# SonSang/dmesh2_renderer

Measured on AMD Instinct MI355X. Metric: Mpixels/s fwd+bwd @1080p/1M tris, higher is better.
Workload: dtype f32

## Files before the change

### dmesh2_renderer_amd/csrc/dm2_binning.hip

```cpp
#include <hip/hip_runtime.h>

#include <cstdlib>
#include <cstring>
#include <rocprim/rocprim.hpp>

#include "dm2_device_math.h"
#include "dm2_pairs.h"
#include "dm2_stage.h"
#include "dm2_state.h"

namespace dm2 {

__global__ void __launch_bounds__(256) k_zero_words(uint32_t* __restrict__ p, int64_t n) {
    const int64_t i = (int64_t)blockIdx.x * blockDim.x + threadIdx.x;
    if (i < n) p[i] = 0u;
}
static void launch_zero_words(void* p, int64_t n, hipStream_t st) {
    if (n > 0) hipLaunchKernelGGL(k_zero_words, dim3((unsigned)((n + 255) / 256)), dim3(256), 0, st, (uint32_t*)p, n);
}

struct TilePlace { uint32_t base; int leader; uint32_t offset; };
__device__ __forceinline__ bool wave_tiles_shared(uint32_t t, bool act) {
    const unsigned long long all = __ballot(act);
    if (all == 0) return false;
    const int l0 = __ffsll((long long)all) - 1;
    const unsigned long long m0 = __ballot(act && t == (uint32_t)__builtin_amdgcn_readlane((int)t, l0));
    return __popcll(m0) * 8 > __popcll(all);
}
template <bool RANK, int STRIDE>
__device__ __forceinline__ TilePlace wave_count_tiles_issue(uint32_t* cnt, uint32_t t, bool act, bool grouped) {
    const int lane = (int)__builtin_amdgcn_mbcnt_hi(~0u, __builtin_amdgcn_mbcnt_lo(~0u, 0u));
    TilePlace p; p.base = 0u; p.leader = lane; p.offset = 0u;
    const unsigned long long all = __ballot(act);
    if (all == 0) return p;
    if (!grouped) {
        if (act) { if (RANK) p.base = atomicAdd(cnt + (int64_t)STRIDE * t, 1u); else atomicAdd(cnt + (int64_t)STRIDE * t, 1u); }
        return p;
    }
    unsigned long long todo = all, mine = 0;
    while (todo) {
        const int l = __ffsll((long long)todo) - 1;
        const uint32_t tl = (uint32_t)__builtin_amdgcn_readlane((int)t, l);
        const unsigned long long m = __ballot(act && t == tl);
        if (act && t == tl) mine = m;
        todo &= ~m;
    }
    p.leader = act ? __ffsll((long long)mine) - 1 : lane;
    if (act && lane == p.leader) {
        if (RANK) p.base = atomicAdd(cnt + (int64_t)STRIDE * t, (uint32_t)__popcll(mine));
        else atomicAdd(cnt + (int64_t)STRIDE * t, (uint32_t)__popcll(mine));
    }
    p.offset = (uint32_t)__popcll(mine & ((1ull << lane) - 1ull));
    return p;
}
__device__ __forceinline__ uint32_t wave_count_tiles_finish(const TilePlace& p) {
    return (uint32_t)__shfl((int)p.base, p.leader) + p.offset;
}
template <bool RANK, int STRIDE>
__device__ __forceinline__ uint32_t wave_count_tiles(uint32_t* cnt, uint32_t t, bool act) {
    const TilePlace p = wave_count_tiles_issue<RANK, STRIDE>(cnt, t, act, wave_tiles_shared(t, act));
    return RANK ? wave_count_tiles_finish(p) : 0u;
}

enum { PRE_LAYERS = 0,
       PRE_FUSED = 1 };
__host__ __device__ constexpr int pre_items(int) { return 1; }

__device__ __forceinline__ void store_records(const FaceRec& r, bool has, unsigned long long tmask, int64_t idx, uint4* __restrict__ recs, uint4* sw) {
    const uint4* src = reinterpret_cast<const uint4*>(&r);
    const int lane = (int)(threadIdx.x & 63);
    uint4* dst = recs + (idx - lane) * FACE_REC_U4;
#pragma unroll
    for (int half = 0; half < 2; half++) {
        if (has) {
#pragma unroll
            for (int k = 0; k < 8; k++) sw[lane * 8 + (k ^ (lane & 7))] = src[half * 8 + k];
        }
        __builtin_amdgcn_fence(__ATOMIC_SEQ_CST, "wavefront");
#pragma unroll
        for (int j = 0; j < 8; j++) {
            const int rr = j * 8 + (lane >> 3), c = lane & 7;
            if ((tmask >> rr) & 1ull) dst[(int64_t)rr * FACE_REC_U4 + half * 8 + c] = sw[rr * 8 + (c ^ (rr & 7))];
        }
        __builtin_amdgcn_fence(__ATOMIC_SEQ_CST, "wavefront");
    }
}

#ifndef DM2_PRE_WAVES
#define DM2_PRE_WAVES 1
#endif
template <int MODE>
__global__ void __launch_bounds__(256, DM2_PRE_WAVES)
k_preprocess(int B, int P, int F, uint32_t gx, uint32_t gy, uint32_t block_stride, const int32_t* __restrict__ patch_min,
             const int32_t* __restrict__ faces, const float* __restrict__ verts_ndc,
             const float* __restrict__ verts_image, FaceState fs, dm2_render_desc d) {
    constexpr bool PACK = MODE == PRE_FUSED;
    constexpr int DM2_PRE_ITEMS = pre_items(MODE);
    const int64_t BF = (int64_t)B * F;
    int64_t idx_[DM2_PRE_ITEMS]; int vid_[DM2_PRE_ITEMS][3]; float2 img_[DM2_PRE_ITEMS][3];
#pragma unroll
    for (int it = 0; it < DM2_PRE_ITEMS; it++) {
        const uint32_t chunk = (uint32_t)(((uint64_t)blockIdx.x * block_stride) % gridDim.x);
        idx_[it] = ((int64_t)chunk * DM2_PRE_ITEMS + it) * 256 + threadIdx.x;
        const int64_t ic = idx_[it] < BF ? idx_[it] : BF - 1;
        const int f = (int)(ic % F);
        vid_[it][0] = faces[3 * f]; vid_[it][1] = faces[3 * f + 1]; vid_[it][2] = faces[3 * f + 2];
    }
#pragma unroll
    for (int it = 0; it < DM2_PRE_ITEMS; it++) {
        const int64_t ic = idx_[it] < BF ? idx_[it] : BF - 1;
        const float* img = verts_image + (ic / F) * P * 2;
#pragma unroll
        for (int k = 0; k < 3; k++) img_[it][k] = *reinterpret_cast<const float2*>(img + 2 * vid_[it][k]);
    }
#pragma unroll
    for (int it = 0; it < DM2_PRE_ITEMS; it++) {
    const bool valid = idx_[it] < BF;
    if (!__ballot(valid)) break;
    const int64_t idx = valid ? idx_[it] : BF - 1;
    const int b = (int)(idx / F), f = (int)(idx % F);
    const uint32_t pmx = patch_min ? (uint32_t)patch_min[2 * b] : 0u, pmy = patch_min ? (uint32_t)patch_min[2 * b + 1] : 0u;
    const int v0 = vid_[it][0], v1 = vid_[it][1], v2 = vid_[it][2];
    const float* ndc = verts_ndc + (int64_t)b * P * 3;
    const float2 i0 = img_[it][0], i1 = img_[it][1], i2 = img_[it][2];

    uint32_t touched = 0, lo = 0, hi = 0;
    float d01 = 0.f, dmin = 0.f, dmax = 0.f;
    {
        uint32_t x0, y0, x1, y1;
        patch_rect_from_tri(pmx, pmy, i0.x, i0.y, i1.x, i1.y, i2.x, i2.y, gx, gy, x0, y0, x1, y1);
        touched = valid ? (y1 - y0) * (x1 - x0) : 0u;
        if (touched != 0) {
            const float z0 = ndc[3 * v0 + 2], z1 = ndc[3 * v1 + 2], z2 = ndc[3 * v2 + 2];
            const float max_z = fmaxf(fmaxf(z0, z1), z2);
            const float min_z = fminf(fminf(z0, z1), z2);
            float depth = ((0.0f + z0) + z1) + z2;
            depth = depth / 3.0f;
            if (max_z < -1.0f || min_z > 1.0f) touched = 0;
            else {
                auto to01 = [](float z) { float d = (z + 1.0f) * 0.5f; if (d < 0.0f) d = 0.0f; if (d > 1.0f) d = 1.0f; return d; };
                d01 = to01(depth); dmin = to01(min_z); dmax = to01(max_z);
                lo = x0 | (y0 << 16); hi = x1 | (y1 << 16);
            }
        }
    }
    const bool small = touched != 0 && touched <= 4;
    const bool any_small = __ballot(small) != 0ull;
    TilePlace place[4];
    {
        const uint32_t x0 = lo & 0xFFFFu, y0 = lo >> 16, x1 = hi & 0xFFFFu;
        const uint32_t tb = (uint32_t)((int64_t)gx * gy * b);
        const bool big = touched > 4;
        if (any_small) {
            const uint32_t w = x1 - x0;
            const bool grouped = wave_tiles_shared(tb + (y0 * gx + x0), small);
#pragma unroll
            for (uint32_t k = 0; k < 4; k++) {
                const uint32_t ky = w == 1 ? k : (w == 2 ? k >> 1 : (w == 3 ? (k == 3 ? 1u : 0u) : 0u)), kx = k - ky * w;
                const bool act = small && k < touched;
                place[k] = wave_count_tiles_issue<true, 1>(fs.tile_cnt, act ? tb + ((y0 + ky) * gx + x0 + kx) : 0u, act, grouped);
            }
        }
        if (__ballot(big)) {
            uint32_t cx = x0, cy = y0;
            for (uint32_t k = 0; ; k++) {
                const bool act = big && k < touched;
                if (!__ballot(act)) break;
                wave_count_tiles<false, 1>(fs.tile_cnt_big, act ? tb + (cy * gx + cx) : 0u, act);
                if (++cx == x1) { cx = x0; cy++; }
            }
        }
    }
    if (MODE != PRE_LAYERS) {
        unsigned long long cand = 0;
        if (touched != 0) {
            float bx0 = fminf(fminf(i0.x, i1.x), i2.x), bx1 = fmaxf(fmaxf(i0.x, i1.x), i2.x);
            float by0 = fminf(fminf(i0.y, i1.y), i2.y), by1 = fmaxf(fmaxf(i0.y, i1.y), i2.y);
            float tx0 = -1.0f, tx1 = 3.0e38f, ty0 = -1.0f, ty1 = 3.0e38f;
            if (!(d.flags & DM2_FLAG_TABLES_FROM_IMAGE)) {
                const float* av = d.aa_face_verts + idx * 6;
                bx0 = fminf(fminf(av[0], av[2]), av[4]); bx1 = fmaxf(fmaxf(av[0], av[2]), av[4]);
                by0 = fminf(fminf(av[1], av[3]), av[5]); by1 = fmaxf(fmaxf(av[1], av[3]), av[5]);
                tx0 = (float)((lo & 0xFFFFu) * TILE) - 1.0f; tx1 = (float)((hi & 0xFFFFu) * TILE);
                ty0 = (float)((lo >> 16) * TILE) - 1.0f; ty1 = (float)((hi >> 16) * TILE);
            }
            if (bx0 == bx0 && bx1 == bx1 && by0 == by0 && by1 == by1) {
                const float Wm = (float)(gx * TILE), Hm = (float)(gy * TILE);
                float lo_x = fminf(fmaxf(ceilf(bx0) - 1.0f - (float)pmx, 0.0f), Wm), hi_x = fminf(fmaxf(floorf(bx1) - (float)pmx, -1.0f), Wm - 1.0f);
                float lo_y = fminf(fmaxf(ceilf(by0) - 1.0f - (float)pmy, 0.0f), Hm), hi_y = fminf(fmaxf(floorf(by1) - (float)pmy, -1.0f), Hm - 1.0f);
                lo_x = fmaxf(lo_x, tx0); hi_x = fminf(hi_x, tx1); lo_y = fmaxf(lo_y, ty0); hi_y = fminf(hi_y, ty1);
                const float w = hi_x - lo_x + 1.0f, h = hi_y - lo_y + 1.0f;
                if (w > 0.0f && h > 0.0f) cand = (unsigned long long)w * (unsigned long long)h;
            }
        }
        const int sa = wave_inclusive_scan((int)(cand & 0xFFFFFFull)), sb = wave_inclusive_scan((int)(cand >> 24));
        const int last = 63 - __clzll((long long)__ballot(true));
        if ((int)(threadIdx.x & 63) == last) {
            const unsigned long long tot = (unsigned long long)(uint32_t)sa + ((unsigned long long)(uint32_t)sb << 24);
            if (tot) atomicAdd(fs.pair_part + ((blockIdx.x * 4 + (threadIdx.x >> 6)) & (PAIR_PARTS - 1)), tot);
        }
    }
    if (valid) fs.tiles_touched[idx] = touched;
    if (touched != 0) {
        fs.depths[idx] = d01; fs.min_depths[idx] = dmin; fs.max_depths[idx] = dmax;
        fs.rect_lo[idx] = lo; fs.rect_hi[idx] = hi;
    }
    if (PACK) {
        __shared__ uint4 s_t[PACK ? 4 : 1][PACK ? 64 * 8 : 1];
        const unsigned long long tmask = __ballot(touched != 0);
        if (tmask != 0ull) {
            FaceRec r;
            if (touched != 0) { pack_face(d, b, f, i1, r); r.pad[0] = 0.f; }
            store_records(r, touched != 0, tmask, idx_[it], fs.recs, s_t[threadIdx.x >> 6]);
        }
    }
    if (any_small) {
        const uint32_t r0 = wave_count_tiles_finish(place[0]), r1 = wave_count_tiles_finish(place[1]);
        const uint32_t r2 = wave_count_tiles_finish(place[2]), r3 = wave_count_tiles_finish(place[3]);
        if (small) fs.tile_rank[idx] = make_uint4(r0, r1, r2, r3);
    }
    __builtin_amdgcn_sched_barrier(0);
    }
}

__global__ void __launch_bounds__(1024)
k_tile_scan(int64_t Tn, const uint32_t* __restrict__ cnt, const uint32_t* __restrict__ cnt_big, uint32_t* __restrict__ start,
            const unsigned long long* __restrict__ pair_part, uint32_t* __restrict__ meta, uint32_t* host_meta, uint32_t host_seq,
            uint2* __restrict__ ranges_to_clear) {
    constexpr int RUN = 8, ROUND = 1024 * RUN;
    __shared__ uint32_t s_c[ROUND + ROUND / 32];
    __shared__ uint32_t s_w[16];
    __shared__ uint32_t s_max;
    __shared__ unsigned long long s_pairs, s_total64;
    const int tid = threadIdx.x, lane = tid & 63, wid = tid >> 6;
    if (tid == 0) { s_max = 0; s_pairs = 0ull; s_total64 = 0ull; }
    unsigned long long pair_sum = pair_part[tid];
    uint32_t carry = 0, mx = 0;
    for (int64_t base = 0; base < Tn; base += ROUND) {
#pragma unroll
        for (int k = 0; k < RUN; k++) {
            const int i = k * 1024 + tid;
            const int64_t t = base + i;
            s_c[i + (i >> 5)] = t < Tn ? cnt[t] + cnt_big[t] : 0u;
        }
        __syncthreads();
        uint32_t c8[RUN], sum = 0;
#pragma unroll
        for (int k = 0; k < RUN; k++) { const int i = tid * RUN + k; c8[k] = s_c[i + (i >> 5)]; sum += c8[k]; mx = mx > c8[k] ? mx : c8[k]; }
        const uint32_t inc = (uint32_t)wave_inclusive_scan((int)sum);
        if (lane == 63) s_w[wid] = inc;
        __syncthreads();
        uint32_t before = 0, total = 0;
        for (int w = 0; w < 16; w++) { const uint32_t v = s_w[w]; if (w < wid) before += v; total += v; }
        uint32_t run = carry + before + inc - sum;
#pragma unroll
        for (int k = 0; k < RUN; k++) { const int i = tid * RUN + k; s_c[i + (i >> 5)] = run; run += c8[k]; }
        carry += total;
        unsigned long long s64 = 0;
#pragma unroll
        for (int k = 0; k < RUN; k++) s64 += c8[k];
#pragma unroll
        for (int o = 32; o >= 1; o >>= 1) s64 += __shfl_xor(s64, o);
        if (lane == 0 && s64) atomicAdd(&s_total64, s64);
        __syncthreads();
#pragma unroll
        for (int k = 0; k < RUN; k++) {
            const int i = k * 1024 + tid;
            const int64_t t = base + i;
            if (t < Tn) {
                start[t] = s_c[i + (i >> 5)];
                if (ranges_to_clear) ranges_to_clear[t] = make_uint2(0u, 0u);
            }
        }
        __syncthreads();
    }
    if (mx) atomicMax(&s_max, mx);
    {
        static_assert(PAIR_PARTS == 1024, "one partial sum per thread of k_tile_scan");
        unsigned long long v = pair_sum;
#pragma unroll
        for (int o = 32; o >= 1; o >>= 1) v += __shfl_xor(v, o);
        if (lane == 0 && v) atomicAdd(&s_pairs, v);
    }
    __syncthreads();
    if (tid == 0) {
        const uint32_t longest = s_total64 > 0x7FFFFFFFull ? 0xFFFFFFFFu : s_max;
        const unsigned long long pairs = s_pairs;
        meta[0] = carry; meta[1] = longest; meta[2] = (uint32_t)pairs; meta[3] = (uint32_t)(pairs >> 32);
        if (host_meta) {
            host_meta[0] = carry; host_meta[1] = longest; host_meta[2] = (uint32_t)pairs; host_meta[3] = (uint32_t)(pairs >> 32);
            __hip_atomic_store(&host_meta[4], host_seq, __ATOMIC_RELEASE, __HIP_MEMORY_SCOPE_SYSTEM);
        }
    }
}

enum { TILE_ORDER_INDEX = 0, TILE_ORDER_TAIL = 1, TILE_ORDER_ALL = 2 };
#ifndef DM2_TILE_ORDER
#define DM2_TILE_ORDER -1
#endif
static int tile_order_mode(int64_t Tn) {
    if (DM2_TILE_ORDER >= 0) return DM2_TILE_ORDER;
    const char* e = getenv("DM2_TILE_ORDER_MODE");
    if (e && *e >= '0' && *e <= '2') return *e - '0';
    return Tn <= 16 * 1024 ? TILE_ORDER_ALL : TILE_ORDER_TAIL;
}
__global__ void __launch_bounds__(1024)
k_tile_order(int64_t Tn, const uint32_t* __restrict__ cnt, const uint32_t* __restrict__ cnt_big, const uint32_t* __restrict__ meta,
             uint32_t* __restrict__ order, int mode) {
    __shared__ uint32_t s_h[257];
    __shared__ uint32_t s_w[16];
    __shared__ uint32_t s_k;
    const int64_t per = (Tn + 7) / 8, t0 = (int64_t)blockIdx.x * per;
    const int64_t n = t0 >= Tn ? 0 : (Tn - t0 < per ? Tn - t0 : per);
    const int tid = threadIdx.x, lane = tid & 63, wid = tid >> 6;
    for (int64_t i = n + tid; i < per; i += 1024) order[t0 + i] = 0xFFFFFFFFu;
    if (!cnt || mode == TILE_ORDER_INDEX) { for (int64_t i = tid; i < n; i += 1024) order[t0 + i] = (uint32_t)(t0 + i); return; }
    const uint32_t mx = meta[1] ? meta[1] : 1u;
    auto cls = [&](int64_t t) { const uint64_t c = (uint64_t)cnt[t] + cnt_big[t]; const uint64_t q = c * 255u / mx; return 255u - (uint32_t)(q > 255u ? 255u : q); };
    if (tid < 257) s_h[tid] = 0;
    if (tid == 0) s_k = 255u;
    __syncthreads();
    for (int64_t i = tid; i < n; i += 1024) atomicAdd(&s_h[cls(t0 + i)], 1u);
    __syncthreads();
    {
        const uint32_t v = tid < 256 ? s_h[tid] : 0u;
        const uint32_t inc = (uint32_t)wave_inclusive_scan((int)v);
        if (tid < 256 && lane == 63) s_w[wid] = inc;
        __syncthreads();
        if (tid < 256) {
            uint32_t before = 0;
            for (int w = 0; w < wid; w++) before += s_w[w];
            s_h[tid] = before + inc - v;
            if (mode == TILE_ORDER_TAIL && (uint64_t)(before + inc) * 4u >= (uint64_t)n * 3u) atomicMin(&s_k, (uint32_t)tid);
        }
    }
    __syncthreads();
    const uint32_t K = s_k;
    __syncthreads();
    uint32_t carry = 0;
    for (int64_t base = 0; base < n; base += 1024) {
        const int64_t i = base + tid;
        const uint32_t c = i < n ? cls(t0 + i) : 0xFFFFFFFFu;
        const bool head = i < n && mode == TILE_ORDER_TAIL && c <= K;
        const unsigned long long m = __ballot(head);
        if (lane == 0) s_w[wid] = (uint32_t)__popcll(m);
        __syncthreads();
        uint32_t before = 0, total = 0;
        for (int w = 0; w < 16; w++) { const uint32_t v = s_w[w]; if (w < wid) before += v; total += v; }
        if (head) order[t0 + carry + before + (uint32_t)__popcll(m & ((1ull << lane) - 1ull))] = (uint32_t)(t0 + i);
        else if (i < n) order[t0 + atomicAdd(&s_h[c], 1u)] = (uint32_t)(t0 + i);
        carry += total;
        __syncthreads();
    }
}

__global__ void __launch_bounds__(256)
k_bin_scatter(int B, int F, uint32_t gx, uint32_t gy, uint32_t block_stride, const float* __restrict__ key_depth, FaceState fs,
              uint2* __restrict__ ranges, uint64_t* __restrict__ keys) {
    const int64_t idx0 = (int64_t)(((uint64_t)blockIdx.x * block_stride) % gridDim.x) * blockDim.x + threadIdx.x;
    const bool valid = idx0 < (int64_t)B * F;
    const int64_t idx = valid ? idx0 : 0;
    const uint32_t touched = valid ? fs.tiles_touched[idx] : 0u;
    if (!__ballot(touched != 0)) return;
    const int b = (int)(idx / F), f = (int)(idx % F);
    const uint32_t lo = fs.rect_lo[idx], hi = fs.rect_hi[idx];
    const uint32_t x0 = lo & 0xFFFFu, y0 = lo >> 16, x1 = hi & 0xFFFFu;
    const uint64_t key = ((uint64_t)__float_as_uint(key_depth[idx]) << 32) | (uint32_t)f;
    const int64_t tile_base = (int64_t)gx * gy * b;
    if (touched != 0 && touched <= 4) {
        const uint4 r4 = fs.tile_rank[idx];
        const uint32_t rk[4] = {r4.x, r4.y, r4.z, r4.w};
        const uint32_t w = x1 - x0;
#pragma unroll
        for (uint32_t k = 0; k < 4; k++) {
            const uint32_t ky = w == 1 ? k : (w == 2 ? k >> 1 : (w == 3 ? (k == 3 ? 1u : 0u) : 0u)), kx = k - ky * w;
            if (k < touched) keys[fs.tile_start[tile_base + ((y0 + ky) * gx + x0 + kx)] + rk[k]] = key;
        }
    }
    const bool big = touched > 4;
    if (__ballot(big)) {
        uint32_t cx = x0, cy = y0;
        for (uint32_t k = 0; ; k++) {
            const bool act = big && k < touched;
            if (!__ballot(act)) break;
            const uint32_t t = act ? (uint32_t)tile_base + (cy * gx + cx) : 0u;
            const uint32_t place = wave_count_tiles<true, 2>(&ranges[0].y, t, act);
            if (act) keys[fs.tile_start[t] + fs.tile_cnt[t] + place] = key;
            if (++cx == x1) { cx = x0; cy++; }
        }
    }
}

constexpr int TILE_SORT_LDS = 2048;
constexpr int TILE_SORT_RANK = 512;
__device__ __forceinline__ void sort_pair_indices(int p, int lk, int lj, int& i, int& j) {
    if (lk) { const int blk = p >> (lk - 1), off = p & ((1 << (lk - 1)) - 1); i = (blk << lk) + off; j = (blk << lk) + ((1 << lk) - 1 - off); }
    else { const int blk = p >> lj, off = p & ((1 << lj) - 1); i = (blk << (lj + 1)) + off; j = i + (1 << lj); }
}
__device__ __forceinline__ void sort_step_sync(bool wave_local_next, bool wave_local_this) {
    if (wave_local_next && wave_local_this) __builtin_amdgcn_fence(__ATOMIC_SEQ_CST, "wavefront");
    else __syncthreads();
}
__global__ void __launch_bounds__(256)
k_tile_sort(int64_t Tn, uint32_t R, const uint32_t* __restrict__ tile_start, uint64_t* __restrict__ keys,
            uint32_t* __restrict__ face_list, uint2* __restrict__ ranges, uint32_t* __restrict__ hit_valid) {
    __shared__ __attribute__((aligned(16))) uint64_t s_key[TILE_SORT_LDS];
    const int64_t t = blockIdx.x;
    const int tid = threadIdx.x;
    const uint32_t s0 = tile_start[t], e0 = (t + 1 < Tn) ? tile_start[t + 1] : R;
    const int n = (int)(e0 - s0);
    if (t == 0 && tid < 8) hit_valid[tid] = 0u;
    if (tid == 0) ranges[t] = n ? make_uint2(s0, e0) : make_uint2(0u, 0u);
    if (n == 0) return;
    uint64_t* const seg = keys + s0;
    int LN = 0;
    while ((1 << LN) < n) LN++;
    const int N = 1 << LN, half = N >> 1;
    if (n <= TILE_SORT_RANK) {
        const int n2 = (n + 1) & ~1;
        for (int i = tid; i < n2; i += 256) s_key[i] = i < n ? seg[i] : ~0ull;
        __syncthreads();
        const uint64_t k0 = tid < n ? s_key[tid] : 0ull, k1 = tid + 256 < n ? s_key[tid + 256] : 0ull;
        int r0 = 0, r1 = 0;
        const ulonglong2* const kk2 = reinterpret_cast<const ulonglong2*>(s_key);
        if (n <= 256) {
            for (int i = 0; i < (n2 >> 1); i++) { const ulonglong2 kk = kk2[i]; r0 += (int)(kk.x < k0) + (int)(kk.y < k0); }
        } else {
            for (int i = 0; i < (n2 >> 1); i++) {
                const ulonglong2 kk = kk2[i];
                r0 += (int)(kk.x < k0) + (int)(kk.y < k0); r1 += (int)(kk.x < k1) + (int)(kk.y < k1);
            }
        }
        if (tid < n) face_list[s0 + r0] = (uint32_t)k0;
        if (tid + 256 < n) face_list[s0 + r1] = (uint32_t)k1;
    } else if (n <= TILE_SORT_LDS) {
        for (int i = tid; i < N; i += 256) s_key[i] = i < n ? seg[i] : ~0ull;
        __syncthreads();
        for (int lk = 1; lk <= LN; lk++) {
            for (int lj = lk - 1; lj >= 0; lj--) {
                const bool mirror = lj == lk - 1;
                for (int p = tid; p < half; p += 256) {
                    int i, j;
                    sort_pair_indices(p, mirror ? lk : 0, lj, i, j);
                    const uint64_t a = s_key[i], c = s_key[j];
                    if (c < a) { s_key[i] = c; s_key[j] = a; }
                }
                const bool this_local = lj + 1 <= 7;
                const bool next_local = lj > 0 ? true : (lk + 1 <= 7);
                sort_step_sync(this_local && next_local, true);
            }
        }
        __syncthreads();
        for (int i = tid; i < n; i += 256) face_list[s0 + i] = (uint32_t)s_key[i];
    } else {
        for (int lk = 1; lk <= LN; lk++) {
            for (int lj = lk - 1; lj >= 0; lj--) {
                const bool mirror = lj == lk - 1;
                for (int p = tid; p < half; p += 256) {
                    int i, j;
                    sort_pair_indices(p, mirror ? lk : 0, lj, i, j);
                    if (j < n) {
                        const uint64_t a = seg[i], c = seg[j];
                        if (c < a) { seg[i] = c; seg[j] = a; }
                    }
                }
                __syncthreads();
            }
        }
        for (int i = tid; i < n; i += 256) face_list[s0 + i] = (uint32_t)seg[i];
    }
}

__global__ void __launch_bounds__(256)
k_emit_keys(int B, int F, uint32_t gx, uint32_t gy, const float* __restrict__ key_depth, FaceState fs,
            uint64_t* __restrict__ keys, uint32_t* __restrict__ vals) {
    const int64_t idx = (int64_t)blockIdx.x * blockDim.x + threadIdx.x;
    if (idx >= (int64_t)B * F) return;
    if (fs.tiles_touched[idx] == 0) return;
    const int b = (int)(idx / F), f = (int)(idx % F);
    uint32_t off = (idx == 0) ? 0u : fs.face_offsets[idx - 1];
    const uint32_t lo = fs.rect_lo[idx], hi = fs.rect_hi[idx];
    const uint32_t x0 = lo & 0xFFFFu, y0 = lo >> 16, x1 = hi & 0xFFFFu, y1 = hi >> 16;
    const uint32_t dbits = __float_as_uint(key_depth[idx]);
    const uint64_t tile_base = (uint64_t)gx * gy * (uint64_t)b;
    for (uint32_t y = y0; y < y1; y++)
        for (uint32_t x = x0; x < x1; x++) {
            const uint64_t key = ((tile_base + (uint64_t)(y * gx + x)) << 32) | dbits;
            keys[off] = key; vals[off] = (uint32_t)f; off++;
        }
}

__global__ void __launch_bounds__(256)
k_tile_ranges(int64_t L, const uint64_t* __restrict__ keys, uint2* __restrict__ ranges, uint32_t* __restrict__ hit_valid) {
    const int64_t idx = (int64_t)blockIdx.x * blockDim.x + threadIdx.x;
    if (idx < 8) hit_valid[idx] = 0u;
    if (idx >= L) return;
    const uint32_t cur = (uint32_t)(keys[idx] >> 32);
    if (idx == 0) ranges[cur].x = 0;
    else {
        const uint32_t prev = (uint32_t)(keys[idx - 1] >> 32);
        if (cur != prev) { ranges[prev].y = (uint32_t)idx; ranges[cur].x = (uint32_t)idx; }
    }
    if (idx == L - 1) ranges[cur].y = (uint32_t)L;
}

static uint32_t higher_msb(uint32_t n) {
    uint32_t msb = sizeof(n) * 4, step = msb;
    while (step > 1) { step /= 2; if (n >> msb) msb += step; else msb -= step; }
    if (n >> msb) msb++;
    return msb;
}

size_t scan_temp_bytes(int64_t BF) {
    thread_local int64_t last_bf = -1; thread_local size_t last_bytes = 0;
    if (BF == last_bf) return last_bytes;
    size_t bytes = 0;
    uint32_t* p = nullptr;
    (void)rocprim::inclusive_scan(nullptr, bytes, p, p, (size_t)(BF > 0 ? BF : 1), rocprim::plus<uint32_t>());
    last_bf = BF; last_bytes = bytes;
    return bytes;
}

unsigned sort_end_bit(int64_t Tn) {
    const unsigned e = 32u + higher_msb((uint32_t)Tn);
    return e > 64u ? 64u : e;
}

size_t sort_temp_bytes(int64_t R, int64_t Tn) {
    thread_local int64_t last_r = -1, last_tn = -1; thread_local size_t last_bytes = 0;
    if (R == last_r && Tn == last_tn) return last_bytes;
    size_t bytes = 0;
    uint64_t* k = nullptr; uint32_t* v = nullptr;
    (void)rocprim::radix_sort_pairs(nullptr, bytes, k, k, v, v, (size_t)(R > 0 ? R : 1), 0u, sort_end_bit(Tn));
    last_r = R; last_tn = Tn; last_bytes = bytes;
    return bytes;
}

void launch_tile_order_identity(int64_t Tn, uint32_t* tile_order, hipStream_t st) {
    if (Tn > 0) hipLaunchKernelGGL(k_tile_order, dim3(8), dim3(1024), 0, st, Tn, nullptr, nullptr, nullptr, tile_order, (int)TILE_ORDER_INDEX);
}

static uint32_t chunk_stride(uint32_t chunks) {
    if (chunks <= 64u) return 1u;
    auto gcd = [](uint32_t a, uint32_t b) { while (b) { const uint32_t t = a % b; a = b; b = t; } return a; };
    uint32_t stride = chunks / 13u + 1u;
    while (gcd(stride, chunks) != 1u) stride++;
    return stride;
}

hipError_t launch_preprocess_scan(int B, int P, int F, int W, int H, const int32_t* patch_min, const int32_t* faces,
                                  const float* verts_ndc, const float* verts_image, FaceState fs, const dm2_render_desc* pack,
                                  uint32_t* host_meta, uint32_t host_seq, uint2* ranges_to_clear, uint32_t* tile_order, hipStream_t st) {
    const int64_t BF = (int64_t)B * F;
    if (BF == 0) return hipSuccess;
    const uint32_t gx = (W + TILE - 1) / TILE, gy = (H + TILE - 1) / TILE;
    const int64_t Tn = (int64_t)B * gx * gy;
    StageTimer tm(ST_PREP, st);
    if (Tn == 0) return hipMemsetAsync(fs.plan_meta, 0, 4 * sizeof(uint32_t), st);
    launch_zero_words(fs.tile_cnt, 2 * Tn + 2 * PAIR_PARTS, st);
    const int mode = pack && fs.recs ? PRE_FUSED : PRE_LAYERS;
    const int blocks = (int)((BF + 256 * pre_items(mode) - 1) / (256 * pre_items(mode)));
    const uint32_t stride = chunk_stride((uint32_t)blocks);
    if (mode == PRE_FUSED)
        hipLaunchKernelGGL(k_preprocess<PRE_FUSED>, dim3(blocks), dim3(256), 0, st, B, P, F, gx, gy, stride, patch_min, faces, verts_ndc, verts_image, fs, *pack);
    else
        hipLaunchKernelGGL(k_preprocess<PRE_LAYERS>, dim3(blocks), dim3(256), 0, st, B, P, F, gx, gy, stride, patch_min, faces, verts_ndc, verts_image, fs,
                           dm2_render_desc{});
    hipLaunchKernelGGL(k_tile_scan, dim3(1), dim3(1024), 0, st, Tn, fs.tile_cnt, fs.tile_cnt_big, fs.tile_start, fs.pair_part, fs.plan_meta,
                       host_meta, host_seq, ranges_to_clear);
    if (tile_order) hipLaunchKernelGGL(k_tile_order, dim3(8), dim3(1024), 0, st, Tn, fs.tile_cnt, fs.tile_cnt_big, fs.plan_meta, tile_order, tile_order_mode(Tn));
    return hipSuccess;
}

hipError_t launch_bin_sort(int B, int F, int W, int H, int64_t R, int64_t max_tile_entries, bool legacy, const float* key_depth,
                           FaceState fs, BinningState bs, uint2* ranges, bool ranges_cleared, uint32_t* tile_order, hipStream_t st) {
    const uint32_t gx = (W + TILE - 1) / TILE, gy = (H + TILE - 1) / TILE;
    const int64_t Tn = (int64_t)B * gx * gy;
    if (!ranges_cleared) launch_zero_words(ranges, 2 * Tn, st);
    if (tile_order && !ranges_cleared)
        hipLaunchKernelGGL(k_tile_order, dim3(8), dim3(1024), 0, st, Tn, R > 0 ? fs.tile_cnt : nullptr, fs.tile_cnt_big, fs.plan_meta, tile_order, tile_order_mode(Tn));
    hipError_t e = hipSuccess;
    if (R <= 0) return e;
    const int64_t BF = (int64_t)B * F;
    if (!legacy && max_tile_entries <= TILE_SORT_MAX) {
        {
            StageTimer tm(ST_EMIT, st);
            hipLaunchKernelGGL(k_bin_scatter, dim3((int)((BF + 255) / 256)), dim3(256), 0, st, B, F, gx, gy, chunk_stride((uint32_t)((BF + 255) / 256)), key_depth, fs, ranges, bs.keys);
        }
        StageTimer tm(ST_SORT, st);
        hipLaunchKernelGGL(k_tile_sort, dim3((unsigned)Tn), dim3(256), 0, st, Tn, (uint32_t)R, fs.tile_start, bs.keys, bs.face_list,
                           ranges, bs.hit_valid);
        return hipSuccess;
    }
    {
        StageTimer tm(ST_EMIT, st);
        size_t bytes = fs.scan_temp_bytes;
        e = rocprim::inclusive_scan(fs.scan_temp, bytes, fs.tiles_touched, fs.face_offsets, (size_t)BF, rocprim::plus<uint32_t>(), st);
        if (e != hipSuccess) return e;
        hipLaunchKernelGGL(k_emit_keys, dim3((int)((BF + 255) / 256)), dim3(256), 0, st, B, F, gx, gy, key_depth, fs,
                           bs.keys_unsorted, bs.face_list_unsorted);
    }
    {
        StageTimer tm(ST_SORT, st);
        size_t bytes = bs.sort_temp_bytes;
        e = rocprim::radix_sort_pairs(bs.sort_temp, bytes, bs.keys_unsorted, bs.keys, bs.face_list_unsorted, bs.face_list,
                                      (size_t)R, 0u, sort_end_bit(Tn), st);
        if (e != hipSuccess) return e;
    }
    StageTimer tm(ST_RANGES, st);
    hipLaunchKernelGGL(k_tile_ranges, dim3((int)((R + 255) / 256)), dim3(256), 0, st, R, bs.keys, ranges, bs.hit_valid);
    return hipSuccess;
}

}
```

Measured before the change: 1223.

## Replace rank-counting tile sort with wave bitonic runs plus merge-rank binary search

```diff
diff --git a/dmesh2_renderer_amd/csrc/dm2_binning.hip b/dmesh2_renderer_amd/csrc/dm2_binning.hip
--- a/dmesh2_renderer_amd/csrc/dm2_binning.hip
+++ b/dmesh2_renderer_amd/csrc/dm2_binning.hip
@@ -401,6 +401,48 @@
     if (wave_local_next && wave_local_this) __builtin_amdgcn_fence(__ATOMIC_SEQ_CST, "wavefront");
     else __syncthreads();
 }
+template <int M>
+__device__ __forceinline__ uint32_t lane_xor(uint32_t v, int lane) {
+    static_assert(M == 1 || M == 2 || M == 3 || M == 4 || M == 7 || M == 8 || M == 15 || M == 16 || M == 31 || M == 32 || M == 63, "no route for this mask");
+    if constexpr (M == 1) return (uint32_t)__builtin_amdgcn_update_dpp(0, (int)v, 0xB1, 0xF, 0xF, true);
+    else if constexpr (M == 2) return (uint32_t)__builtin_amdgcn_update_dpp(0, (int)v, 0x4E, 0xF, 0xF, true);
+    else if constexpr (M == 3) return (uint32_t)__builtin_amdgcn_update_dpp(0, (int)v, 0x1B, 0xF, 0xF, true);
+    else if constexpr (M == 7) return (uint32_t)__builtin_amdgcn_update_dpp(0, (int)v, 0x141, 0xF, 0xF, true);
+    else if constexpr (M == 15) return (uint32_t)__builtin_amdgcn_update_dpp(0, (int)v, 0x140, 0xF, 0xF, true);
+    else if constexpr (M == 8) return (uint32_t)__builtin_amdgcn_update_dpp(0, (int)v, 0x128, 0xF, 0xF, true);
+    else if constexpr (M == 32) {
+        const auto r = __builtin_amdgcn_permlane32_swap(v, v, false, false);
+        return lane < 32 ? r[1] : r[0];
+    }
+    else if constexpr (M == 63) return lane_xor<32>(lane_xor<31>(v, lane), lane);
+    else return (uint32_t)__builtin_amdgcn_ds_swizzle((int)v, 0x1F | (M << 10));
+}
+template <int M, int K>
+__device__ __forceinline__ void run_exchange(uint64_t (&k)[K], int lane) {
+    constexpr int HB = M >= 32 ? 32 : M >= 16 ? 16 : M >= 8 ? 8 : M >= 4 ? 4 : M >= 2 ? 2 : 1;
+    const bool upper = (lane & HB) != 0;
+#pragma unroll
+    for (int c = 0; c < K; c++) {
+        const uint64_t o = ((uint64_t)lane_xor<M>((uint32_t)(k[c] >> 32), lane) << 32) | lane_xor<M>((uint32_t)k[c], lane);
+        k[c] = (o < k[c]) != upper ? o : k[c];
+    }
+}
+template <int K>
+__device__ __forceinline__ void sort_runs(uint64_t (&k)[K], int lane) {
+    run_exchange<1, K>(k, lane);
+    run_exchange<3, K>(k, lane); run_exchange<1, K>(k, lane);
+    run_exchange<7, K>(k, lane); run_exchange<2, K>(k, lane); run_exchange<1, K>(k, lane);
+    run_exchange<15, K>(k, lane); run_exchange<4, K>(k, lane); run_exchange<2, K>(k, lane); run_exchange<1, K>(k, lane);
+    run_exchange<31, K>(k, lane); run_exchange<8, K>(k, lane); run_exchange<4, K>(k, lane); run_exchange<2, K>(k, lane); run_exchange<1, K>(k, lane);
+    run_exchange<63, K>(k, lane); run_exchange<16, K>(k, lane); run_exchange<8, K>(k, lane); run_exchange<4, K>(k, lane); run_exchange<2, K>(k, lane);
+    run_exchange<1, K>(k, lane);
+}
+__device__ __forceinline__ int run_lower_bound(const uint64_t* run, uint64_t key) {
+    int pos = 0;
+#pragma unroll
+    for (int s = 32; s >= 1; s >>= 1) pos += run[pos + s - 1] < key ? s : 0;
+    return pos + (run[pos] < key ? 1 : 0);
+}
 __global__ void __launch_bounds__(256)
 k_tile_sort(int64_t Tn, uint32_t R, const uint32_t* __restrict__ tile_start, uint64_t* __restrict__ keys,
             uint32_t* __restrict__ face_list, uint2* __restrict__ ranges, uint32_t* __restrict__ hit_valid) {
@@ -417,22 +459,41 @@
     while ((1 << LN) < n) LN++;
     const int N = 1 << LN, half = N >> 1;
     if (n <= TILE_SORT_RANK) {
-        const int n2 = (n + 1) & ~1;
-        for (int i = tid; i < n2; i += 256) s_key[i] = i < n ? seg[i] : ~0ull;
-        __syncthreads();
-        const uint64_t k0 = tid < n ? s_key[tid] : 0ull, k1 = tid + 256 < n ? s_key[tid + 256] : 0ull;
-        int r0 = 0, r1 = 0;
-        const ulonglong2* const kk2 = reinterpret_cast<const ulonglong2*>(s_key);
+        const int lane = tid & 63, wid = tid >> 6;
+        if (n <= 64) {
+            if (wid) return;
+            uint64_t k[1] = {lane < n ? seg[lane] : ~0ull};
+            sort_runs<1>(k, lane);
+            if (lane < n) face_list[s0 + lane] = (uint32_t)k[0];
+            return;
+        }
+        const int nruns = (n + 63) >> 6;
         if (n <= 256) {
-            for (int i = 0; i < (n2 >> 1); i++) { const ulonglong2 kk = kk2[i]; r0 += (int)(kk.x < k0) + (int)(kk.y < k0); }
+            const int i0 = wid * 64 + lane;
+            uint64_t k[1] = {i0 < n ? seg[i0] : ~0ull};
+            if (wid < nruns) { sort_runs<1>(k, lane); s_key[i0] = k[0]; }
+            __syncthreads();
+            if (wid >= nruns) return;
+            int rank = lane;
+            for (int r = 0; r < nruns; r++)
+                if (r != wid) rank += run_lower_bound(s_key + r * 64, k[0]);
+            if (i0 < n) face_list[s0 + rank] = (uint32_t)k[0];
         } else {
-            for (int i = 0; i < (n2 >> 1); i++) {
-                const ulonglong2 kk = kk2[i];
-                r0 += (int)(kk.x < k0) + (int)(kk.y < k0); r1 += (int)(kk.x < k1) + (int)(kk.y < k1);
-            }
-        }
-        if (tid < n) face_list[s0 + r0] = (uint32_t)k0;
-        if (tid + 256 < n) face_list[s0 + r1] = (uint32_t)k1;
+            const int i0 = wid * 64 + lane, i1 = i0 + 256;
+            uint64_t k[2] = {seg[i0], i1 < n ? seg[i1] : ~0ull};
+            const bool two = wid + 4 < nruns;
+            if (two) { sort_runs<2>(k, lane); s_key[i1] = k[1]; }
+            else { uint64_t k0[1] = {k[0]}; sort_runs<1>(k0, lane); k[0] = k0[0]; }
+            s_key[i0] = k[0];
+            __syncthreads();
+            int rank0 = lane, rank1 = lane;
+            for (int r = 0; r < nruns; r++) {
+                if (r != wid) rank0 += run_lower_bound(s_key + r * 64, k[0]);
+                if (two && r != wid + 4) rank1 += run_lower_bound(s_key + r * 64, k[1]);
+            }
+            face_list[s0 + rank0] = (uint32_t)k[0];
+            if (i1 < n) face_list[s0 + rank1] = (uint32_t)k[1];
+        }
     } else if (n <= TILE_SORT_LDS) {
         for (int i = tid; i < N; i += 256) s_key[i] = i < n ? seg[i] : ~0ull;
         __syncthreads();
```

New measurement: 1234, median of 4. No clear change (+0.9%).
